# dordanino12/unet-convlstm

Hardware: AMD Instinct MI355X
Metric: training frames/sec, Moving-MNIST 64x64 seq-20 (higher is better)
Workload: dtype bf16; 1 GPU; TemporalUNetDualView(base_ch=64, use_skip_lstm=True) train step, 64x64 seq-20, per-GPU batch 32, AdamW+clip; global_batch=32, seq_len=20, parallelism=dp1

## Files before the change

include/uclstm.h:

```cpp
#ifndef UCLSTM_H
#define UCLSTM_H

#include <stdint.h>

#ifdef __cplusplus
extern "C" {
#endif

#define UCLSTM_ABI_VERSION 16

#define UCLSTM_OK            0
#define UCLSTM_E_BADARG     -1
#define UCLSTM_E_LAUNCH     -2
#define UCLSTM_E_NODEVICE   -3

#define UCLSTM_ACT_TYPE_BF16 0
#define UCLSTM_ACT_TYPE_F16  1


typedef struct {
    const void* ptr;
    int32_t C;
    int32_t Hs, Ws;
    int32_t offY, offX;
// ... 156 lines not shown

int32_t uclstm_bn_bwd_param_grads(const float* sums, int32_t groups, int32_t Cp, int32_t C, float* dgamma, float* dbeta,
                                  int32_t accumulate, void* stream);

int32_t uclstm_maxpool2_fwd(const void* a, void* p, int32_t n_img, int32_t H, int32_t W, int32_t Cp, void* stream);
int32_t uclstm_maxpool2_bwd(const void* a, const void* dp, const void* add, void* da, int32_t n_img, int32_t H, int32_t W, int32_t Cp,
                            void* stream);

int32_t uclstm_splitk_finish(const float* pre, int32_t nslab, int64_t slab, int32_t ld, const float* bias, const float* col_scale,
                             const float* col_shift, int32_t relu, void* out, int64_t pixels, int32_t C, void* stream);

int32_t uclstm_lstm_bwd_pointwise(const void* gates, const float* c_prev, const float* c_new,
                                  const void* dh_a, const void* dh_b, int32_t dh_b_is_f32 ,
                                  int32_t dh_b_nslab , int64_t dh_b_slab ,
                                  float* dc_io, int32_t dc_is_zero, void* dgates, int64_t pixels, int32_t Hd_p, void* stream);
int32_t uclstm_lstm_fwd_pointwise(float* pre, int32_t nslab ,
                                  int64_t slab ,
                                  int32_t clear ,
                                  const float* pre_add ,
                                  const float* bias, const float* c_prev, float* c_out, void* h_out,
                                  void* gates_out, int64_t pixels, int32_t Hd_p, void* stream);
typedef struct {
    float* pre;
    const float* pre_add;
    const float* bias;
    const float* c_prev;
    float* c_out;
    void* h_out;
    void* gates_out;
    int64_t slab;
// ... 154 lines not shown
```

unet-convlstm_amd/_lib.py:

```python
from __future__ import annotations

import ctypes as C
import os
import re

import torch

HERE = os.path.dirname(os.path.abspath(__file__))
LIB_PATH = os.environ.get("UCLSTM_LIB") or os.path.join(HERE, "libuclstm.so")
HEADER_PATH = os.path.join(HERE, "..", "include", "uclstm.h")

ABI_VERSION = 16
EPI_STORE, EPI_LSTM, EPI_ATOMIC = 0, 1, 2
NMODE_IDENTITY, NMODE_LSTM, NMODE_TAPMAJOR = 0, 1, 2
KMODE_IDENTITY, KMODE_GATES, KMODE_IM2COL = 0, 1, 2
ACT_TYPE_BF16, ACT_TYPE_F16 = 0, 1

_ERRORS = {-1: "bad argument (shape/alignment/null contract)", -2: "kernel launch failed", -3: "no gfx950 device"}


class UclstmError(RuntimeError):
    pass


# ... 24 lines not shown

class WgradDesc(C.Structure):
    _fields_ = [("n_img", C.c_int32), ("H", C.c_int32), ("W", C.c_int32),
                ("ktap", C.c_int32), ("scale", C.c_int32), ("pad", C.c_int32), ("nsrc", C.c_int32),
                ("src", Src * 2),
                ("N", C.c_int32), ("Ktot", C.c_int32),
                ("nseg", C.c_int32), ("seg", Seg * 4),
                ("dwp", C.c_void_p), ("splits", C.c_int32), ("accumulate", C.c_int32), ("overlapped", C.c_int32), ("reserved_", C.c_int32),
                ("slab", C.c_int64)]


class LstmFwdPwArgs(C.Structure):
    _fields_ = [("pre", C.c_void_p), ("pre_add", C.c_void_p), ("bias", C.c_void_p), ("c_prev", C.c_void_p), ("c_out", C.c_void_p),
                ("h_out", C.c_void_p), ("gates_out", C.c_void_p), ("slab", C.c_int64), ("pixels", C.c_int64),
                ("nslab", C.c_int32), ("clear", C.c_int32), ("Hd_p", C.c_int32), ("reserved_", C.c_int32)]


class PackDesc(C.Structure):
    _fields_ = [("N", C.c_int32), ("Ktot", C.c_int32), ("taps", C.c_int32), ("nsrc", C.c_int32),
                ("kseg", C.c_int32 * 2), ("cvalid", C.c_int32 * 2), ("choff", C.c_int32 * 2),
                ("n_mode", C.c_int32), ("n_valid", C.c_int32), ("n_cp", C.c_int32),
                ("k_mode", C.c_int32), ("k_hdp", C.c_int32), ("k_hd", C.c_int32),
                ("tap_flip", C.c_int32),
                ("stride_n", C.c_int64), ("stride_k", C.c_int64), ("stride_tap", C.c_int64),
                ("stride_ntap", C.c_int64)]


class PackJob(C.Structure):
    _fields_ = [("d", PackDesc), ("w", C.c_void_p), ("wp", C.c_void_p),
                ("block0", C.c_int32), ("nblocks", C.c_int32), ("gx", C.c_int32), ("family", C.c_int32),
# ... 48 lines not shown
    "uclstm_bn_bwd_apply": [_P, _P, _P, _P, _P, _P, _P, _P, _L, _L, _I, _P],
    "uclstm_bn_pool_bwd_rows": [_L, _I, _I, _I, _I],
    "uclstm_bn_apply_relu_pool": [_P, _P, _P, _P, _P, _L, _I, _I, _I, _I, _P],
    "uclstm_bn_pool_bwd_reduce": [_P, _P, _P, _P, _P, _P, _P, _P, _P, _L, _I, _I, _I, _I, _P],
    "uclstm_bn_pool_bwd_apply": [_P, _P, _P, _P, _P, _P, _P, _P, _P, _L, _I, _I, _I, _I, _P],
    "uclstm_bn_head_fwd": [_P, _P, _P, _P, _P, _P, _L, _L, _I, _I, _P],
    "uclstm_bn_head_bwd_reduce": [_P, _P, _P, _P, _P, _P, _P, _P, _P, _P, _P, _L, _L, _I, _I, _P],
    "uclstm_bn_head_bwd_reduce_ordered": [_P, _P, _P, _P, _P, _P, _P, _P, _P, _P, _P, _P, _L, _L, _I, _I, _I, _P],
    "uclstm_bn_head_bwd_apply": [_P, _P, _P, _P, _P, _P, _P, _P, _P, _L, _L, _I, _I, _P],
    "uclstm_bn_bwd_param_grads": [_P, _I, _I, _I, _P, _P, _I, _P],
    "uclstm_maxpool2_fwd": [_P, _P, _I, _I, _I, _I, _P],
    "uclstm_maxpool2_bwd": [_P, _P, _P, _P, _I, _I, _I, _I, _P],
    "uclstm_lstm_bwd_pointwise": [_P, _P, _P, _P, _P, _I, _I, _L, _P, _I, _P, _L, _I, _P],
    "uclstm_lstm_fwd_pointwise": [_P, _I, _L, _I, _P, _P, _P, _P, _P, _P, _L, _I, _P],
    "uclstm_lstm_fwd_pointwise_group": [C.POINTER(LstmFwdPwArgs), _I, _P],
    "uclstm_splitk_finish": [_P, _I, _L, _I, _P, _P, _P, _I, _P, _L, _I, _P],
    "uclstm_nchw_to_nhwc": [_P, _P, _I, _I, _I, _I, _I, _I, _L, _L, _P],
    "uclstm_nhwc_to_nchw": [_P, _P, _I, _I, _I, _I, _I, _P],
    "uclstm_nchw_grad_to_nhwc": [_P, _P, _I, _I, _I, _I, _I, _P],
    "uclstm_im2col3x3_first": [_P, _P, _I, _I, _I, _I, _I, _I, _L, _L, _P],
    "uclstm_nchw_to_nhwc_f32": [_P, _P, _I, _I, _I, _I, _I, _P],
    "uclstm_nhwc_to_nchw_f32": [_P, _P, _I, _I, _I, _I, _I, _P],
    "uclstm_outconv_fwd": [_P, _P, _P, _P, _L, _I, _I, _I, _I, _P],
    "uclstm_outconv_bwd": [_P, _P, _P, _P, _P, _P, _L, _I, _I, _I, _I, _P],
    "uclstm_outconv_bwd_ordered_rows": [_L, _I],
    "uclstm_outconv_bwd_ordered": [_P, _P, _P, _P, _P, _P, _P, _I, _L, _I, _I, _I, _I, _I, _P],
    "uclstm_colsum": [_P, _P, _L, _I, _P],
    "uclstm_colsum_ordered_rows": [_L, _I],
    "uclstm_colsum_ordered": [_P, _P, _P, _L, _I, _I, _I, _P],
    "uclstm_ordered_sum_f32": [_P, _I, _I, _P, _I, _P],
# ... 107 lines not shown
```

unet-convlstm_amd/csrc/igemm_fwd.hip:

```cpp
#include "common.h"
#include <cstdlib>
#include <type_traits>

namespace {

constexpr int BK = 64;

constexpr uint32_t OOB = 0x80000000u;

struct Derived {
    int Mg;
    int tpg;
    int n_mtiles;
    int n_ntiles;
    int kseg0, kseg1;
    int ksteps;
    int ksplit;
    int kper;
    FastDiv dHW, dW;
    FastDiv dPHW, dW2;
    uint32_t xbias[2];
    uint32_t xbytes[2];
    uint32_t wbytes;
    int strip;
// ... 598 lines not shown
    int n;
    int first[GROUP_MAX + 1];
    int nblk[GROUP_MAX];
    uclstm_igemm_desc d[GROUP_MAX];
    Derived dv[GROUP_MAX];
};

template <int NSRC>
__global__ __launch_bounds__(Shape<2>::NT, 1) void igemm_fwd_group_kernel(const FwdGroup g) {
    const int b = (int)blockIdx.x;
#define UCLSTM_GROUP_MEMBER(j_)                                                                            \
    if (j_ < g.n && b >= g.first[j_] && b < g.first[j_ + 1]) {                                             \
        const int bid = b - g.first[j_];                                                                   \
        if (bid >= g.nblk[j_]) return;                                                                     \
        if (g.d[j_].epi == UCLSTM_EPI_LSTM) igemm_fwd_body<UCLSTM_EPI_LSTM, 2, NSRC>(g.d[j_], g.dv[j_], bid);   \
        else igemm_fwd_body<UCLSTM_EPI_ATOMIC, 2, NSRC>(g.d[j_], g.dv[j_], bid);                           \
        return;                                                                                            \
    }
    UCLSTM_GROUP_MEMBER(0)
    UCLSTM_GROUP_MEMBER(1)
    UCLSTM_GROUP_MEMBER(2)
    UCLSTM_GROUP_MEMBER(3)
#undef UCLSTM_GROUP_MEMBER
}


constexpr int C64_WBYTES = 9 * 64 * 128;
constexpr int C64_ROW = 66 * 128;
constexpr int C64_SLOTS = 10;
constexpr int C64_RED = C64_WBYTES + C64_SLOTS * C64_ROW;
constexpr int C64_SMEM = C64_RED + 4 * 64 * 2 * 4;
// ... 460 lines not shown

static int32_t fwd_group_run(const uclstm_igemm_desc* descs, int32_t n, void* stream, int query) {
    if (!descs || n < 1 || n > GROUP_MAX) return UCLSTM_E_BADARG;
    FwdGroup g{};
    int64_t work[GROUP_MAX];
    int order[GROUP_MAX];
    Derived dvs[GROUP_MAX];
    int64_t nblks[GROUP_MAX];
    for (int i = 0; i < n; ++i) {
        const uclstm_igemm_desc& d = descs[i];
        int shp = 0;
        int64_t mg = 0;
        const int32_t rc = plan_fwd(d, dvs[i], shp, nblks[i], mg);
        if (rc != UCLSTM_OK) return rc;
        if (shp != 2 || (c64_ok(d) && mg % 256 == 0)) return UCLSTM_E_BADARG;
        if (d.epi != UCLSTM_EPI_LSTM && d.epi != UCLSTM_EPI_ATOMIC) return UCLSTM_E_BADARG;
        if (d.nsrc != descs[0].nsrc) return UCLSTM_E_BADARG;
        work[i] = dvs[i].kper;
        order[i] = i;
    }
    for (int a = 1; a < n; ++a)
        for (int b = a; b > 0 && work[order[b]] > work[order[b - 1]]; --b) { const int t = order[b]; order[b] = order[b - 1]; order[b - 1] = t; }
    g.n = n;
    int64_t at = 0;
    for (int k = 0; k < n; ++k) {
        const int i = order[k];
        g.first[k] = (int)at;
        g.nblk[k] = (int)nblks[i];
        g.d[k] = descs[i];
        g.dv[k] = dvs[i];
        at += (nblks[i] + 7) / 8 * 8;
// ... 21 lines not shown
```

unet-convlstm_amd/csrc/pointwise.hip:

```cpp
#include "common.h"
#include <algorithm>
#include <cstdlib>

namespace {

constexpr int NT = 256;

__device__ __forceinline__ void unpack8(const uint4 u, float (&f)[8]) {
    Pack16 p;
    p.u = u;
#pragma unroll
    for (int i = 0; i < 8; ++i) f[i] = act_to_f32(p.e[i]);
}
__device__ __forceinline__ uint4 pack8(const float (&f)[8]) {
    Pack16 p;
#pragma unroll
    for (int i = 0; i < 8; ++i) p.e[i] = f32_to_act(f[i]);
    return p.u;
}
__device__ __forceinline__ float act16_product(float a, float b) {
    float p = a * b;
#ifdef UCLSTM_ACT_F16
    asm("" : "+v"(p));
#endif
// ... 1008 lines not shown
    FastDiv dq[PW_GROUP_MAX];
};
__global__ void lstm_fwd_pw_group_kernel(const LstmFwdPwGroup g) {
    const int b = (int)blockIdx.x;
#pragma unroll
    for (int j = 0; j < PW_GROUP_MAX; ++j) {
        if (j < g.n && b >= g.first[j] && b < g.first[j + 1]) {
            const uclstm_lstm_fwd_pw_args& a = g.a[j];
            lstm_fwd_pw_body(a.pre, a.nslab, a.slab, a.clear, a.pre_add, a.bias, a.c_prev, a.c_out, (act16*)a.h_out, (act16*)a.gates_out,
                             a.pixels * (a.Hd_p / 4), g.dq[j], a.Hd_p, 64 * ((a.Hd_p + 15) / 16), b - g.first[j], g.first[j + 1] - g.first[j]);
            return;
        }
    }
}

__global__ void nchw_to_nhwc_kernel(const float* __restrict__ x, uint4* __restrict__ out, int64_t items, int C, int cpc, FastDiv dHW,
                                    FastDiv dcpc, FastDiv dinner, int64_t inner_stride, int64_t outer_stride) {
    const int HW = dHW.d;
    for (int64_t idx = (int64_t)blockIdx.x * NT + threadIdx.x; idx < items; idx += (int64_t)gridDim.x * NT) {
        const uint32_t t = fdiv((uint32_t)idx, dHW);
        const uint32_t pix = (uint32_t)idx - t * HW;
        const uint32_t img = fdiv(t, dcpc);
        const uint32_t cc = t - img * cpc;
        const uint32_t o = fdiv(img, dinner);
        const uint32_t in = img - o * dinner.d;
        const float* src = x + (int64_t)in * outer_stride + (int64_t)o * inner_stride;
        float v[8];
#pragma unroll
        for (int i = 0; i < 8; ++i) {
            const int c = cc * 8 + i;
// ... 847 lines not shown
                  (act16*)gates_out, items, make_fastdiv(Hd_p / 4), Hd_p, N);
    return UCLSTM_OK;
}

extern "C" int32_t uclstm_lstm_bwd_pointwise(const void* gates, const float* c_prev, const float* c_new, const void* dh_a,
                                             const void* dh_b, int32_t dh_b_is_f32, int32_t dh_b_nslab, int64_t dh_b_slab, float* dc_io,
                                             int32_t dc_is_zero, void* dgates, int64_t pixels, int32_t Hd_p, void* stream) {
    if (!lstm_bwd_pw_ok(gates, c_prev, c_new, dh_a, dh_b, dh_b_is_f32, dh_b_nslab, dh_b_slab, dc_io, dgates, pixels, Hd_p)) return UCLSTM_E_BADARG;
    const int64_t chunks = pixels * (Hd_p / 8);
    UCLSTM_LAUNCH(lstm_bwd_pw_kernel, dim3(ew_grid(chunks)), dim3(NT), 0, (hipStream_t)stream, (const uint4*)gates, c_prev, c_new,
                       (const uint4*)dh_a, dh_b, dh_b_is_f32, dh_b_nslab, dh_b_slab, dc_io, dc_is_zero, (uint4*)dgates, chunks,
                       make_fastdiv(Hd_p / 8));
    return UCLSTM_OK;
}

extern "C" int32_t uclstm_nchw_to_nhwc(const float* x, void* out, int32_t n_img, int32_t C, int32_t Cp, int32_t H, int32_t W,
                                       int32_t inner, int64_t inner_stride, int64_t outer_stride, void* stream) {
    if (!x || !aligned16(out) || n_img <= 0 || C <= 0 || Cp < C || (Cp % 8) || H <= 0 || W <= 0 || inner <= 0 || (n_img % inner))
        return UCLSTM_E_BADARG;
    const int64_t items = (int64_t)n_img * (Cp / 8) * H * W;
    if (items >= ((int64_t)1 << 31)) return UCLSTM_E_BADARG;
    UCLSTM_LAUNCH(nchw_to_nhwc_kernel, dim3(ew_grid(items)), dim3(NT), 0, (hipStream_t)stream, x, (uint4*)out, items, C, Cp / 8,
                       make_fastdiv(H * W), make_fastdiv(Cp / 8), make_fastdiv(inner), inner_stride, outer_stride);
    return UCLSTM_OK;
}

extern "C" int32_t uclstm_nchw_grad_to_nhwc(const float* g, void* out, int32_t n_img, int32_t C, int32_t Cp, int32_t H, int32_t W,
                                            void* stream) {
    return uclstm_nchw_to_nhwc(g, out, n_img, C, Cp, H, W, n_img, 0, (int64_t)C * H * W, stream);
}
// ... 278 lines not shown
```

unet-convlstm_amd/modules.py:

```python
from __future__ import annotations

from typing import List, Optional, Sequence, Tuple

import torch
import torch.nn as nn

from . import ops
from ._lib import UclstmError

Tensor = torch.Tensor


def _need_grad(*ts) -> bool:
    return torch.is_grad_enabled() and any(t is not None and t.requires_grad for t in ts)


class ConvLSTMCell(nn.Module):

    def __init__(self, input_dim, hidden_dim, kernel_size=3, bias=True):
        super().__init__()
        if kernel_size % 2 == 0 or not 1 <= kernel_size <= 7:
            raise UclstmError("ConvLSTMCell: kernel_size must be odd and <= 7")
        padding = kernel_size // 2
        self.input_dim = input_dim
# ... 292 lines not shown
            st = []
            for s in state:
                if s is None or s[0] is None:
                    st.append(None)
                else:
                    st.append((ops.ToNHWC.apply(s[0].contiguous().float()), ops.StateToNHWC.apply(s[1].contiguous().float())))
        grouped = False
        if self.use_skip_lstm and len(self.temporal.layers) == 1:
            cells = (self.temporal.layers[0], self.lstm_skip3.layers[0], self.lstm_skip2.layers[0])
            h0, c0 = (None, None) if (st is None or st[0] is None) else st[0]
            members = [(seq(xb), h0, c0), (seq(x3), None, None), (seq(x2), None, None)]
            full = [(xs, hh, cc, cl.conv.weight, cl.conv.bias, cl.hidden_dim, cl.input_dim) for (xs, hh, cc), cl in zip(members, cells)]
            if ops.convlstm_group_ok(full):
                needs = [_need_grad(*f[:5]) for f in full]
                pre = ops.convlstm_group_forward(full, any(needs))
                outs = [ops.ConvLSTMSeqPre.apply(*f, nd, hh, ch, gt) for f, nd, (hh, ch, gt) in zip(full, needs, pre)]
                b_all, new_st = outs[0][0], [(outs[0][0][-1], outs[0][1])]
                x3_l, x2_l = outs[1][0], outs[2][0]
                grouped = True
        if not grouped:
            b_all, new_st = self.temporal.seq_nhwc(seq(xb), st)
            if self.use_skip_lstm:
                x3_l, _ = self.lstm_skip3.seq_nhwc(seq(x3), None)
                x2_l, _ = self.lstm_skip2.seq_nhwc(seq(x2), None)
        if self.use_skip_lstm:
            x3 = x3_l.reshape(T * B, *x3_l.shape[2:])
            x2 = x2_l.reshape(T * B, *x2_l.shape[2:])
        b_flat = b_all.reshape(T * B, *b_all.shape[2:])

        d3 = self.up3.forward_nhwc(b_flat, x3, c * 8, T)
        d2 = self.up2.forward_nhwc(d3, x2, c * 4, T)
# ... 48 lines not shown
```

unet-convlstm_amd/ops.py:

```python
from __future__ import annotations

import ctypes as C
import os
from typing import List, Optional, Sequence, Tuple

import torch

from . import _lib as L

BF16 = torch.bfloat16
F16 = torch.float16
F32 = torch.float32
ACT = (BF16, F16)

_COMPUTE_DTYPE = BF16


def set_compute_dtype(dtype) -> None:
    global _COMPUTE_DTYPE
    if dtype not in ACT:
        raise L.UclstmError(f"compute dtype must be torch.bfloat16 or torch.float16, got {dtype}")
    _COMPUTE_DTYPE = dtype


# ... 128 lines not shown
    return C.c_void_p(torch.cuda.current_stream().cuda_stream)


def _dev(t: torch.Tensor, dtype=None, what: str = "tensor") -> torch.Tensor:
    if not isinstance(t, torch.Tensor) or not t.is_cuda:
        raise L.UclstmError(f"{what}: a HIP device tensor is required (this package has no CPU path)")
    if dtype is not None and (t.dtype not in dtype if isinstance(dtype, tuple) else t.dtype != dtype):
        raise L.UclstmError(f"{what}: expected {dtype}, got {t.dtype}")
    if not t.is_contiguous():
        raise L.UclstmError(f"{what}: must be contiguous")
    return t


def _p(t: Optional[torch.Tensor]):
    return None if t is None else C.c_void_p(t.data_ptr())


PROFILE: Optional[list] = None


SHAPE_LOG: Optional[list] = None
KERNEL_LOG: Optional[list] = None


LAUNCH_LOG: Optional[list] = None


def _log_shape(d) -> None:
    if SHAPE_LOG is not None or KERNEL_LOG is not None or LAUNCH_LOG is not None:
        shp = int(L.lib.uclstm_igemm_fwd_shape(C.byref(d)))
# ... 498 lines not shown


def _schedule_join(device) -> None:
    key = str(device)
    if key in _JOIN_PENDING:
        return
    _JOIN_PENDING.add(key)

    def join():
        _JOIN_PENDING.discard(key)
        torch.cuda.current_stream(device).wait_stream(side_stream(device))

    torch.autograd.Variable._execution_engine.queue_callback(join)


def wgrad_into_param(weight: torch.Tensor, desc: L.PackDesc, inputs: Sequence[torch.Tensor], run_gemm) -> Optional[torch.Tensor]:
    g = weight.grad
    if not (ASYNC_WGRAD and g is not None and g.dtype == F32 and g.is_contiguous() and g.shape == weight.shape):
        return unpack_wgrad(desc, run_gemm(), weight)
    dev = weight.device
    main, side = torch.cuda.current_stream(dev), side_stream(dev)
    side.wait_stream(main)
    global _WGRAD_OVERLAPPED
    with torch.cuda.stream(side):
        _WGRAD_OVERLAPPED = True
        try:
            dwp = run_gemm()
        finally:
            _WGRAD_OVERLAPPED = False
        _unpack_wgrad_launch(desc, dwp, g, 1)
        for t in inputs:
            if t is not None:
                t.record_stream(side)
# ... 201 lines not shown

def igemm_group(items, K, kind: str = "igemm_fwd_group") -> None:
    arr = (L.IgemmDesc * len(items))(*[it[0] for it in items])
    for it in items:
        _log_shape(it[0])
    _timed(kind + "[patch128x256]" if PROFILE is not None else kind, sum(it[1] for it in items),
           lambda: L.check(K.uclstm_igemm_fwd_group(arr, len(items), _stream()), "igemm_fwd_group"),
           " | ".join(it[3] for it in items), nbytes=sum(it[2] for it in items))


def group_launchable(descs) -> bool:
    arr = (L.IgemmDesc * len(descs))(*descs)
    return int(L.lib.uclstm_igemm_fwd_group_blocks(arr, len(descs))) > 0


def igemm_wgrad(srcs: Sequence[SrcView], dy_segs, N: int, Ktot: int, out_hw: Tuple[int, int], n_img: int, *, ktap: int, scale: int = 1,
                pad: int = 0) -> torch.Tensor:
    dev = srcs[0].t.device
    _same_act_dtype([sv.t for sv in srcs] + [sg[0] for sg in dy_segs], "igemm_wgrad")
    K = _k(srcs[0].t)
    per_img = max([_bytes_per_img(sv.t) for sv in srcs] + [_bytes_per_img(sg[0]) for sg in dy_segs])
    chunks = _img_chunks(n_img, 1, per_img, "igemm_wgrad")
    descs = []
    for i0, i1 in chunks:
        d = L.WgradDesc()
        d.n_img, d.H, d.W = i1 - i0, out_hw[0], out_hw[1]
        d.ktap, d.scale, d.pad, d.nsrc = ktap, scale, pad, len(srcs)
        for i, sv in enumerate(srcs):
            (sv if len(chunks) == 1 else SrcView(sv.t[i0:i1], sv.offY, sv.offX)).fill(d.src[i])
        d.N, d.Ktot = N, Ktot
        d.nseg = len(dy_segs)
        for i, sg in enumerate(dy_segs):
            _fill_seg(d.seg[i], *(sg if len(chunks) == 1 else (sg[0][i0:i1],) + tuple(sg[1:])))
        d.splits, d.accumulate, d.slab = 0, 1, N * Ktot
        d.overlapped = int(_WGRAD_OVERLAPPED)
        splits = int(L.lib.uclstm_igemm_wgrad_splits(C.byref(d)))
        if splits < 1:
            raise L.UclstmError(f"igemm_wgrad: bad descriptor (code {splits})")
        d.splits = splits
        descs.append(d)
    if LAUNCH_LOG is not None:
        if len(chunks) > 1:
            LAUNCH_LOG.append(("split", "igemm_wgrad", len(chunks)))
        for d in descs:
            LAUNCH_LOG.append(("wgrad", int(L.lib.uclstm_igemm_wgrad_shape(C.byref(d))), N, Ktot, int(d.splits)))
    total = sum(d.splits for d in descs)
    dwp = torch.empty((total, N, Ktot), dtype=F32, device=dev)
    taps = ktap * ktap
    at = 0
    for d in descs:
        d.dwp = dwp[at].data_ptr()
        at += d.splits
        flops = 2.0 * d.n_img * out_hw[0] * out_hw[1] * N * taps * sum(s.t.shape[3] for s in srcs)
        kind = "igemm_wgrad"
        if PROFILE is not None:
            kind += "[" + {4: "ring64", 3: "p3_256x256", 2: "p2_128x128", 1: "p2_64x256", 0: "generic"}.get(int(L.lib.uclstm_igemm_wgrad_shape(C.byref(d))), "?") + "]"
        _timed(kind, flops, lambda d=d: L.check(K.uclstm_igemm_wgrad(C.byref(d), _stream()), "igemm_wgrad"),
               f"M={d.n_img * out_hw[0] * out_hw[1]} N={N} K={Ktot} ktap={ktap} splits={d.splits}",
               nbytes=(_nb(*[sv.t for sv in srcs], *[sg[0] for sg in dy_segs]) * (d.n_img / n_img) + 4.0 * N * Ktot) if PROFILE is not None else 0.0)
    return dwp


def colsum(a: torch.Tensor, into: Optional[torch.Tensor] = None) -> torch.Tensor:
    _dev(a, ACT, "colsum input")
    Cp = a.shape[-1]
    if _DETERMINISTIC:
        pixels = a.numel() // Cp
        out = into if into is not None else torch.empty((Cp,), dtype=F32, device=a.device)
        partials = torch.empty((int(L.lib.uclstm_colsum_ordered_rows(pixels, Cp)), Cp), dtype=F32, device=a.device)
        _log_reduce("colsum_ordered")
        L.check(L.lib.uclstm_colsum_ordered(_p(a), _p(partials), _p(out), pixels, Cp, 1 if into is not None else 0, L.act_type(a.dtype),
                                            _stream()), "colsum_ordered")
        return out
    out = into if into is not None else torch.zeros((Cp,), dtype=F32, device=a.device)
# ... 585 lines not shown
        N, H, W, Cp = x.shape
        k = weight.shape[-1]
        dx = torch.empty_like(x)
        scratch = torch.empty((3 * N * H * W + 2,), dtype=F32, device=x.device)
        need_w = ctx.needs_input_grad[1]
        g = direct_grad(weight) if need_w else None
        dw = g if g is not None else (torch.empty_like(weight) if need_w else None)
        L.check(_k(x).uclstm_attention_bwd(_p(x), _p(dout), _p(weight), _p(att), _p(desc), _p(arg), _p(dx), _p(dw), int(g is not None),
                                           _p(scratch), N, H, W, Cp, ctx.channels, k, _stream()), "attention_bwd")
        if g is not None:
            grad_written(weight)
            return dx, None, None
        return dx, dw, None


class ConvLSTMSeq(torch.autograd.Function):

    @staticmethod
    def forward(ctx, x_all, h0, c0, weight, bias, Hd, Cx, need_grad, out=None):
        ctx.set_materialize_grads(False)
        _dev(x_all, ACT, "x_all")
        adt = x_all.dtype
        K = _k(x_all)
        T, B, H, W, Cxp = x_all.shape
        Hdp = cpad(Hd)
        dev = x_all.device
        ks = weight.shape[-1]
        pd = lstm_pack_desc(Hd, Cx, ks)
        bp = pack_bias(pd, bias) if bias is not None else None
        if out is not None:
# ... 84 lines not shown
        need_h0 = ctx.needs_input_grad[1]
        for t in range(T - 1, -1, -1):
            c_prev = c_hist[t] if (has_c0 or t > 0) else None
            L.check(K.uclstm_lstm_bwd_pointwise(_p(gates[t]), _p(c_prev), _p(c_hist[t + 1]),
                                                    _p(dh_all[t]) if dh_all is not None else None, _p(dh_rec),
                                                    1 if ksplit > 1 else 0, nsl, pixels * Hdp, _p(dc),
                                                    int(dc_zero), _p(dgates[t]), pixels, Hdp, _stream()), "lstm_bwd_pointwise")
            dc_zero = False
            if t > 0 or need_h0:
                dh_rec = buf[t & 1]
                if ksplit > 1:
                    igemm_atomic([SrcView(dgates[t])], wd_h, (H, W), B, dh_rec.view(nsl, pixels, Hdp), ksplit, ktap=ks, pad=ks // 2,
                                 slabs=True)
                else:
                    igemm_store([SrcView(dgates[t])], wd_h, (H, W), B, [(dh_rec, 0, ddh.N, 0, 1, 0, 0)], ktap=ks, pad=ks // 2)
        dg_flat = dgates.view(T * B, H, W, 4 * Hdp)
        x_flat = x_all.reshape(T * B, H, W, Cxp)
        hprev_flat = h_hist[:T].reshape(T * B, H, W, Hdp)
        dweight = None
        if ctx.needs_input_grad[3]:
            ud = lstm_wgrad_unpack_desc(Hd, Cx, ks)
            dweight = wgrad_into_param(weight, ud, [x_all, h_hist, dgates],
                                       lambda: igemm_wgrad([SrcView(x_flat), SrcView(hprev_flat)], [(dg_flat, 0, 4 * Hdp, 0, 1, 0, 0)],
                                                           ud.N, ud.Ktot, (H, W), T * B, ktap=ks, pad=ks // 2))
        dbias = None
        if has_bias and ctx.needs_input_grad[4]:
            if Hdp == Hd:
                dbias = bias_grad_from_colsum(dg_flat, bias, 4 * Hd)
            else:
                dbias = colsum(dg_flat).view(4, Hdp)[:, :Hd].reshape(4 * Hd).contiguous()
        dx_all = None
        if ctx.needs_input_grad[0]:
            ddx = lstm_dgrad_pack_desc(Hd, Cx, Cx, ks)
            wd_x = pack_weights(ddx, weight, 0, adt)
            dx_all = torch.empty_like(x_all)
            igemm_store([SrcView(dg_flat)], wd_x, (H, W), T * B, [(dx_all.view(T * B, H, W, Cxp), 0, ddx.N, 0, 1, 0, 0)], ktap=ks,
                        pad=ks // 2)
        dh0 = (dh_rec if dh_rec.dtype == adt else dh_rec.sum(dim=0).to(adt)) if need_h0 else None
        dc0 = dc if (has_c0 and ctx.needs_input_grad[2]) else None
        return dx_all, dh0, dc0, dweight, dbias, None, None, None


GROUP_LSTM = os.environ.get("UCLSTM_GROUP_LSTM", "1") != "0"
FUSE_POOL = os.environ.get("UCLSTM_FUSE_POOL", "1") != "0"
FUSE_HEAD = os.environ.get("UCLSTM_FUSE_HEAD", "1") != "0"
_GROUP_PLANS: dict = {}
_CUS = 256
_BLOCK_OVERHEAD_STEPS = 12.0


def _lpt_makespan(blocks: List[Tuple[float, int]], cus: int = _CUS) -> float:
    import heapq
    free = [0.0] * cus
    for dur, cnt in sorted(blocks, reverse=True):
# ... 138 lines not shown
    @staticmethod
    def forward(ctx, x_all, h0, c0, weight, bias, Hd, Cx, need_grad, h_hist, c_hist, gates):
        ctx.set_materialize_grads(False)
        T = x_all.shape[0]
        if need_grad:
            ctx.save_for_backward(x_all, weight, h_hist, c_hist, gates, bias)
            ctx.cfg = (Hd, Cx, c0 is not None, bias is not None, weight.shape[-1])
            note_use(weight, bias)
        return h_hist[1:], c_hist[T]

    @staticmethod
    def backward(ctx, dh_all, dc_T):
        return ConvLSTMSeq.backward(ctx, dh_all, dc_T) + (None, None, None)


def convlstm_group_ok(members) -> bool:
    if not GROUP_LSTM or len(members) < 2 or len(members) > 4:
        return False
    x0 = members[0][0]
    try:
        descs = []
        for x_all, h0, c0, weight, bias, Hd, Cx in members:
            if x_all.dim() != 5 or x_all.shape[0] != x0.shape[0] or x_all.shape[1] != x0.shape[1] or x_all.dtype != x0.dtype:
                return False
            if weight.shape[-1] != 3 or cpad(Hd) != Hd or Hd % 64 or x_all.shape[4] % 64 or (x_all.shape[1] * x_all.shape[2] * x_all.shape[3]) % 256:
                return False
            T, B, H, W, Cxp = x_all.shape
            pd = lstm_pack_desc(Hd, Cx, 3)
            d = L.IgemmDesc()
            d.n_img, d.H, d.W, d.groups = B, H, W, 1
# ... 52 lines not shown
```

Baseline: 20510 frames/s.

## Group ConvLSTM backward across layers with batched pointwise, dh igemm, and chunked overlapped wgrad

Adds a grouped backward autograd function for the ConvLSTM layers that were already grouped in forward. At each timestep it runs one combined pointwise-backward kernel for all members and one grouped igemm (with store or atomic split-K epilogues) for the recurrent dh. It also launches weight-gradient GEMMs in time chunks on a side stream as the dgates for each chunk become ready. The aim is fewer per-timestep launches and overlap of wgrad with the serial recurrence, at the cost of more complex scheduling, stream synchronization and extra scratch memory.

```diff
diff --git a/include/uclstm.h b/include/uclstm.h
--- a/include/uclstm.h
+++ b/include/uclstm.h
@@ -194,6 +194,19 @@
                                   const void* dh_a, const void* dh_b, int32_t dh_b_is_f32 ,
                                   int32_t dh_b_nslab , int64_t dh_b_slab ,
                                   float* dc_io, int32_t dc_is_zero, void* dgates, int64_t pixels, int32_t Hd_p, void* stream);
+typedef struct {
+    const void* gates;
+    const float* c_prev;
+    const float* c_new;
+    const void* dh_a;
+    const void* dh_b;
+    float* dc_io;
+    void* dgates;
+    int64_t dh_b_slab;
+    int64_t pixels;
+    int32_t dh_b_is_f32, dh_b_nslab, dc_is_zero, Hd_p;
+} uclstm_lstm_bwd_pw_args;
+int32_t uclstm_lstm_bwd_pointwise_group(const uclstm_lstm_bwd_pw_args* args, int32_t n, int32_t act_type, void* stream);
 int32_t uclstm_lstm_fwd_pointwise(float* pre, int32_t nslab ,
                                   int64_t slab ,
                                   int32_t clear ,
diff --git a/unet-convlstm_amd/_lib.py b/unet-convlstm_amd/_lib.py
--- a/unet-convlstm_amd/_lib.py
+++ b/unet-convlstm_amd/_lib.py
@@ -62,6 +62,12 @@
     _fields_ = [("pre", C.c_void_p), ("pre_add", C.c_void_p), ("bias", C.c_void_p), ("c_prev", C.c_void_p), ("c_out", C.c_void_p),
                 ("h_out", C.c_void_p), ("gates_out", C.c_void_p), ("slab", C.c_int64), ("pixels", C.c_int64),
                 ("nslab", C.c_int32), ("clear", C.c_int32), ("Hd_p", C.c_int32), ("reserved_", C.c_int32)]
+
+
+class LstmBwdPwArgs(C.Structure):
+    _fields_ = [("gates", C.c_void_p), ("c_prev", C.c_void_p), ("c_new", C.c_void_p), ("dh_a", C.c_void_p), ("dh_b", C.c_void_p),
+                ("dc_io", C.c_void_p), ("dgates", C.c_void_p), ("dh_b_slab", C.c_int64), ("pixels", C.c_int64),
+                ("dh_b_is_f32", C.c_int32), ("dh_b_nslab", C.c_int32), ("dc_is_zero", C.c_int32), ("Hd_p", C.c_int32)]
 
 
 class PackDesc(C.Structure):
@@ -140,6 +146,7 @@
     "uclstm_lstm_bwd_pointwise": [_P, _P, _P, _P, _P, _I, _I, _L, _P, _I, _P, _L, _I, _P],
     "uclstm_lstm_fwd_pointwise": [_P, _I, _L, _I, _P, _P, _P, _P, _P, _P, _L, _I, _P],
     "uclstm_lstm_fwd_pointwise_group": [C.POINTER(LstmFwdPwArgs), _I, _P],
+    "uclstm_lstm_bwd_pointwise_group": [C.POINTER(LstmBwdPwArgs), _I, _I, _P],
     "uclstm_splitk_finish": [_P, _I, _L, _I, _P, _P, _P, _I, _P, _L, _I, _P],
     "uclstm_nchw_to_nhwc": [_P, _P, _I, _I, _I, _I, _I, _I, _L, _L, _P],
     "uclstm_nhwc_to_nchw": [_P, _P, _I, _I, _I, _I, _I, _P],
diff --git a/unet-convlstm_amd/csrc/igemm_fwd.hip b/unet-convlstm_amd/csrc/igemm_fwd.hip
--- a/unet-convlstm_amd/csrc/igemm_fwd.hip
+++ b/unet-convlstm_amd/csrc/igemm_fwd.hip
@@ -636,7 +636,9 @@
         const int bid = b - g.first[j_];                                                                   \
         if (bid >= g.nblk[j_]) return;                                                                     \
         if (g.d[j_].epi == UCLSTM_EPI_LSTM) igemm_fwd_body<UCLSTM_EPI_LSTM, 2, NSRC>(g.d[j_], g.dv[j_], bid);   \
-        else igemm_fwd_body<UCLSTM_EPI_ATOMIC, 2, NSRC>(g.d[j_], g.dv[j_], bid);                           \
+        else if (NSRC == 1 && g.d[j_].epi == UCLSTM_EPI_STORE) {                                           \
+            if constexpr (NSRC == 1) igemm_fwd_body<UCLSTM_EPI_STORE, 2, 1>(g.d[j_], g.dv[j_], bid);       \
+        } else igemm_fwd_body<UCLSTM_EPI_ATOMIC, 2, NSRC>(g.d[j_], g.dv[j_], bid);                         \
         return;                                                                                            \
     }
     UCLSTM_GROUP_MEMBER(0)
@@ -1127,7 +1129,8 @@
         const int32_t rc = plan_fwd(d, dvs[i], shp, nblks[i], mg);
         if (rc != UCLSTM_OK) return rc;
         if (shp != 2 || (c64_ok(d) && mg % 256 == 0)) return UCLSTM_E_BADARG;
-        if (d.epi != UCLSTM_EPI_LSTM && d.epi != UCLSTM_EPI_ATOMIC) return UCLSTM_E_BADARG;
+        const bool store_ok = d.epi == UCLSTM_EPI_STORE && d.nsrc == 1 && !d.stats;
+        if (d.epi != UCLSTM_EPI_LSTM && d.epi != UCLSTM_EPI_ATOMIC && !store_ok) return UCLSTM_E_BADARG;
         if (d.nsrc != descs[0].nsrc) return UCLSTM_E_BADARG;
         work[i] = dvs[i].kper;
         order[i] = i;
diff --git a/unet-convlstm_amd/csrc/pointwise.hip b/unet-convlstm_amd/csrc/pointwise.hip
--- a/unet-convlstm_amd/csrc/pointwise.hip
+++ b/unet-convlstm_amd/csrc/pointwise.hip
@@ -1046,6 +1046,26 @@
     }
 }
 
+struct LstmBwdPwGroup {
+    int n;
+    int first[PW_GROUP_MAX + 1];
+    uclstm_lstm_bwd_pw_args a[PW_GROUP_MAX];
+    FastDiv dcpc[PW_GROUP_MAX];
+};
+__global__ void lstm_bwd_pw_group_kernel(const LstmBwdPwGroup g) {
+    const int b = (int)blockIdx.x;
+#pragma unroll
+    for (int j = 0; j < PW_GROUP_MAX; ++j) {
+        if (j < g.n && b >= g.first[j] && b < g.first[j + 1]) {
+            const uclstm_lstm_bwd_pw_args& a = g.a[j];
+            lstm_bwd_pw_body((const uint4*)a.gates, a.c_prev, a.c_new, (const uint4*)a.dh_a, a.dh_b, a.dh_b_is_f32, a.dh_b_nslab, a.dh_b_slab,
+                             a.dc_io, a.dc_is_zero, (uint4*)a.dgates, a.pixels * (a.Hd_p / 8), g.dcpc[j], b - g.first[j],
+                             g.first[j + 1] - g.first[j]);
+            return;
+        }
+    }
+}
+
 __global__ void nchw_to_nhwc_kernel(const float* __restrict__ x, uint4* __restrict__ out, int64_t items, int C, int cpc, FastDiv dHW,
                                     FastDiv dcpc, FastDiv dinner, int64_t inner_stride, int64_t outer_stride) {
     const int HW = dHW.d;
@@ -1923,6 +1943,45 @@
     return UCLSTM_OK;
 }
 
+__attribute__((visibility("hidden"))) int32_t UCLSTM_ACT_IMPL(lstm_bwd_pointwise_group)(const uclstm_lstm_bwd_pw_args* args, int32_t n,
+                                                                                       void* stream) {
+    if (!args || n < 1 || n > PW_GROUP_MAX) return UCLSTM_E_BADARG;
+    int order[PW_GROUP_MAX];
+    for (int i = 0; i < n; ++i) {
+        const uclstm_lstm_bwd_pw_args& a = args[i];
+        if (!lstm_bwd_pw_ok(a.gates, a.c_prev, a.c_new, a.dh_a, a.dh_b, a.dh_b_is_f32, a.dh_b_nslab, a.dh_b_slab, a.dc_io, a.dgates, a.pixels,
+                            a.Hd_p))
+            return UCLSTM_E_BADARG;
+        order[i] = i;
+    }
+    for (int x = 1; x < n; ++x)
+        for (int y = x; y > 0 && args[order[y]].pixels * (args[order[y]].Hd_p / 8) > args[order[y - 1]].pixels * (args[order[y - 1]].Hd_p / 8); --y) {
+            const int t = order[y]; order[y] = order[y - 1]; order[y - 1] = t;
+        }
+    LstmBwdPwGroup g{};
+    g.n = n;
+    int64_t at = 0;
+    for (int k = 0; k < n; ++k) {
+        const uclstm_lstm_bwd_pw_args& a = args[order[k]];
+        g.a[k] = a;
+        g.dcpc[k] = make_fastdiv(a.Hd_p / 8);
+        g.first[k] = (int)at;
+        at += ew_grid(a.pixels * (a.Hd_p / 8));
+    }
+    if (at > 0x7fffffff) return UCLSTM_E_BADARG;
+    for (int k = n; k <= PW_GROUP_MAX; ++k) g.first[k] = (int)at;
+    UCLSTM_LAUNCH(lstm_bwd_pw_group_kernel, dim3((unsigned)at), dim3(NT), 0, (hipStream_t)stream, g);
+    return UCLSTM_OK;
+}
+#ifndef UCLSTM_ACT_F16
+int32_t lstm_bwd_pointwise_group_impl_f16(const uclstm_lstm_bwd_pw_args*, int32_t, void*);
+extern "C" int32_t uclstm_lstm_bwd_pointwise_group(const uclstm_lstm_bwd_pw_args* args, int32_t n, int32_t act_type, void* stream) {
+    if (act_type == UCLSTM_ACT_TYPE_BF16) return UCLSTM_ACT_IMPL(lstm_bwd_pointwise_group)(args, n, stream);
+    if (act_type == UCLSTM_ACT_TYPE_F16) return lstm_bwd_pointwise_group_impl_f16(args, n, stream);
+    return UCLSTM_E_BADARG;
+}
+#endif
+
 extern "C" int32_t uclstm_nchw_to_nhwc(const float* x, void* out, int32_t n_img, int32_t C, int32_t Cp, int32_t H, int32_t W,
                                        int32_t inner, int64_t inner_stride, int64_t outer_stride, void* stream) {
     if (!x || !aligned16(out) || n_img <= 0 || C <= 0 || Cp < C || (Cp % 8) || H <= 0 || W <= 0 || inner <= 0 || (n_img % inner))
diff --git a/unet-convlstm_amd/modules.py b/unet-convlstm_amd/modules.py
--- a/unet-convlstm_amd/modules.py
+++ b/unet-convlstm_amd/modules.py
@@ -330,7 +330,10 @@
             if ops.convlstm_group_ok(full):
                 needs = [_need_grad(*f[:5]) for f in full]
                 pre = ops.convlstm_group_forward(full, any(needs))
-                outs = [ops.ConvLSTMSeqPre.apply(*f, nd, hh, ch, gt) for f, nd, (hh, ch, gt) in zip(full, needs, pre)]
+                if all(needs):
+                    outs = ops.convlstm_group_apply(full, pre)
+                else:
+                    outs = [ops.ConvLSTMSeqPre.apply(*f, nd, hh, ch, gt) for f, nd, (hh, ch, gt) in zip(full, needs, pre)]
                 b_all, new_st = outs[0][0], [(outs[0][0][-1], outs[0][1])]
                 x3_l, x2_l = outs[1][0], outs[2][0]
                 grouped = True
diff --git a/unet-convlstm_amd/ops.py b/unet-convlstm_amd/ops.py
--- a/unet-convlstm_amd/ops.py
+++ b/unet-convlstm_amd/ops.py
@@ -166,6 +166,16 @@
 
 def _p(t: Optional[torch.Tensor]):
     return None if t is None else C.c_void_p(t.data_ptr())
+
+
+POISON_SCRATCH = os.environ.get("UCLSTM_POISON_SCRATCH", "0") == "1"
+
+
+def _scratch(shape, dtype, device) -> torch.Tensor:
+    t = torch.empty(shape, dtype=dtype, device=device)
+    if POISON_SCRATCH:
+        t.fill_(float("nan"))
+    return t
 
 
 PROFILE: Optional[list] = None
@@ -694,9 +704,14 @@
     torch.autograd.Variable._execution_engine.queue_callback(join)
 
 
+def wgrad_goes_to_side(weight: torch.Tensor) -> bool:
+    g = weight.grad
+    return bool(ASYNC_WGRAD and g is not None and g.dtype == F32 and g.is_contiguous() and g.shape == weight.shape)
+
+
 def wgrad_into_param(weight: torch.Tensor, desc: L.PackDesc, inputs: Sequence[torch.Tensor], run_gemm) -> Optional[torch.Tensor]:
     g = weight.grad
-    if not (ASYNC_WGRAD and g is not None and g.dtype == F32 and g.is_contiguous() and g.shape == weight.shape):
+    if not wgrad_goes_to_side(weight):
         return unpack_wgrad(desc, run_gemm(), weight)
     dev = weight.device
     main, side = torch.cuda.current_stream(dev), side_stream(dev)
@@ -928,50 +943,78 @@
     return int(L.lib.uclstm_igemm_fwd_group_blocks(arr, len(descs))) > 0
 
 
-def igemm_wgrad(srcs: Sequence[SrcView], dy_segs, N: int, Ktot: int, out_hw: Tuple[int, int], n_img: int, *, ktap: int, scale: int = 1,
-                pad: int = 0) -> torch.Tensor:
-    dev = srcs[0].t.device
+class _WgradPlan:
+    pass
+
+
+def wgrad_plan(srcs: Sequence[SrcView], dy_segs, N: int, Ktot: int, out_hw: Tuple[int, int], ranges: Sequence[Tuple[int, int]], *, ktap: int,
+               scale: int = 1, pad: int = 0, overlapped: Optional[bool] = None) -> _WgradPlan:
     _same_act_dtype([sv.t for sv in srcs] + [sg[0] for sg in dy_segs], "igemm_wgrad")
-    K = _k(srcs[0].t)
     per_img = max([_bytes_per_img(sv.t) for sv in srcs] + [_bytes_per_img(sg[0]) for sg in dy_segs])
-    chunks = _img_chunks(n_img, 1, per_img, "igemm_wgrad")
-    descs = []
-    for i0, i1 in chunks:
-        d = L.WgradDesc()
-        d.n_img, d.H, d.W = i1 - i0, out_hw[0], out_hw[1]
-        d.ktap, d.scale, d.pad, d.nsrc = ktap, scale, pad, len(srcs)
-        for i, sv in enumerate(srcs):
-            (sv if len(chunks) == 1 else SrcView(sv.t[i0:i1], sv.offY, sv.offX)).fill(d.src[i])
-        d.N, d.Ktot = N, Ktot
-        d.nseg = len(dy_segs)
-        for i, sg in enumerate(dy_segs):
-            _fill_seg(d.seg[i], *(sg if len(chunks) == 1 else (sg[0][i0:i1],) + tuple(sg[1:])))
-        d.splits, d.accumulate, d.slab = 0, 1, N * Ktot
-        d.overlapped = int(_WGRAD_OVERLAPPED)
-        splits = int(L.lib.uclstm_igemm_wgrad_splits(C.byref(d)))
-        if splits < 1:
-            raise L.UclstmError(f"igemm_wgrad: bad descriptor (code {splits})")
-        d.splits = splits
-        descs.append(d)
-    if LAUNCH_LOG is not None:
-        if len(chunks) > 1:
-            LAUNCH_LOG.append(("split", "igemm_wgrad", len(chunks)))
+    n_all = srcs[0].t.shape[0]
+    pl = _WgradPlan()
+    pl.srcs, pl.dy_segs, pl.N, pl.Ktot, pl.out_hw, pl.ktap = list(srcs), list(dy_segs), N, Ktot, out_hw, ktap
+    pl.K, pl.dev, pl.n_img, pl.dwp = _k(srcs[0].t), srcs[0].t.device, sum(i1 - i0 for i0, i1 in ranges), None
+    pl.ranges = []
+    for r0, r1 in ranges:
+        chunks = [(r0 + i0, r0 + i1) for i0, i1 in _img_chunks(r1 - r0, 1, per_img, "igemm_wgrad")]
+        descs = []
+        for i0, i1 in chunks:
+            whole = i0 == 0 and i1 == n_all
+            d = L.WgradDesc()
+            d.n_img, d.H, d.W = i1 - i0, out_hw[0], out_hw[1]
+            d.ktap, d.scale, d.pad, d.nsrc = ktap, scale, pad, len(srcs)
+            for i, sv in enumerate(srcs):
+                (sv if whole else SrcView(sv.t[i0:i1], sv.offY, sv.offX)).fill(d.src[i])
+            d.N, d.Ktot = N, Ktot
+            d.nseg = len(dy_segs)
+            for i, sg in enumerate(dy_segs):
+                _fill_seg(d.seg[i], *(sg if whole else (sg[0][i0:i1],) + tuple(sg[1:])))
+            d.splits, d.accumulate, d.slab = 0, 1, N * Ktot
+            d.overlapped = int(_WGRAD_OVERLAPPED if overlapped is None else overlapped)
+            splits = int(L.lib.uclstm_igemm_wgrad_splits(C.byref(d)))
+            if splits < 1:
+                raise L.UclstmError(f"igemm_wgrad: bad descriptor (code {splits})")
+            d.splits = splits
+            descs.append(d)
+        if LAUNCH_LOG is not None:
+            if len(chunks) > 1:
+                LAUNCH_LOG.append(("split", "igemm_wgrad", len(chunks)))
+            for d in descs:
+                LAUNCH_LOG.append(("wgrad", int(L.lib.uclstm_igemm_wgrad_shape(C.byref(d))), N, Ktot, int(d.splits)))
+        pl.ranges.append(descs)
+    pl.total = sum(d.splits for descs in pl.ranges for d in descs)
+    return pl
+
+
+def wgrad_alloc(pl: _WgradPlan) -> torch.Tensor:
+    pl.dwp = _scratch((pl.total, pl.N, pl.Ktot), F32, pl.dev)
+    at = 0
+    for descs in pl.ranges:
         for d in descs:
-            LAUNCH_LOG.append(("wgrad", int(L.lib.uclstm_igemm_wgrad_shape(C.byref(d))), N, Ktot, int(d.splits)))
-    total = sum(d.splits for d in descs)
-    dwp = torch.empty((total, N, Ktot), dtype=F32, device=dev)
-    taps = ktap * ktap
-    at = 0
-    for d in descs:
-        d.dwp = dwp[at].data_ptr()
-        at += d.splits
+            d.dwp = pl.dwp[at].data_ptr()
+            at += d.splits
+    return pl.dwp
+
+
+def wgrad_launch_range(pl: _WgradPlan, i: int) -> None:
+    taps = pl.ktap * pl.ktap
+    srcs, dy_segs, N, Ktot, out_hw = pl.srcs, pl.dy_segs, pl.N, pl.Ktot, pl.out_hw
+    for d in pl.ranges[i]:
         flops = 2.0 * d.n_img * out_hw[0] * out_hw[1] * N * taps * sum(s.t.shape[3] for s in srcs)
         kind = "igemm_wgrad"
         if PROFILE is not None:
             kind += "[" + {4: "ring64", 3: "p3_256x256", 2: "p2_128x128", 1: "p2_64x256", 0: "generic"}.get(int(L.lib.uclstm_igemm_wgrad_shape(C.byref(d))), "?") + "]"
-        _timed(kind, flops, lambda d=d: L.check(K.uclstm_igemm_wgrad(C.byref(d), _stream()), "igemm_wgrad"),
-               f"M={d.n_img * out_hw[0] * out_hw[1]} N={N} K={Ktot} ktap={ktap} splits={d.splits}",
-               nbytes=(_nb(*[sv.t for sv in srcs], *[sg[0] for sg in dy_segs]) * (d.n_img / n_img) + 4.0 * N * Ktot) if PROFILE is not None else 0.0)
+        _timed(kind, flops, lambda d=d: L.check(pl.K.uclstm_igemm_wgrad(C.byref(d), _stream()), "igemm_wgrad"),
+               f"M={d.n_img * out_hw[0] * out_hw[1]} N={N} K={Ktot} ktap={pl.ktap} splits={d.splits}",
+               nbytes=(_nb(*[sv.t for sv in srcs], *[sg[0] for sg in dy_segs]) * (d.n_img / srcs[0].t.shape[0]) + 4.0 * N * Ktot) if PROFILE is not None else 0.0)
+
+
+def igemm_wgrad(srcs: Sequence[SrcView], dy_segs, N: int, Ktot: int, out_hw: Tuple[int, int], n_img: int, *, ktap: int, scale: int = 1,
+                pad: int = 0) -> torch.Tensor:
+    pl = wgrad_plan(srcs, dy_segs, N, Ktot, out_hw, [(0, n_img)], ktap=ktap, scale=scale, pad=pad)
+    dwp = wgrad_alloc(pl)
+    wgrad_launch_range(pl, 0)
     return dwp
 
 
@@ -1587,6 +1630,38 @@
         return dx, dw, None
 
 
+def _lstm_bwd_finish(x_all, weight, bias, h_hist, dgates, dh_rec, dc, cfg, needs, weight_done: bool = False):
+    Hd, Cx, has_c0, has_bias, ks = cfg
+    T, B, H, W, Cxp = x_all.shape
+    Hdp = cpad(Hd)
+    adt = x_all.dtype
+    dg_flat = dgates.view(T * B, H, W, 4 * Hdp)
+    x_flat = x_all.reshape(T * B, H, W, Cxp)
+    hprev_flat = h_hist[:T].reshape(T * B, H, W, Hdp)
+    dweight = None
+    if needs[3] and not weight_done:
+        ud = lstm_wgrad_unpack_desc(Hd, Cx, ks)
+        dweight = wgrad_into_param(weight, ud, [x_all, h_hist, dgates],
+                                   lambda: igemm_wgrad([SrcView(x_flat), SrcView(hprev_flat)], [(dg_flat, 0, 4 * Hdp, 0, 1, 0, 0)],
+                                                       ud.N, ud.Ktot, (H, W), T * B, ktap=ks, pad=ks // 2))
+    dbias = None
+    if has_bias and needs[4]:
+        if Hdp == Hd:
+            dbias = bias_grad_from_colsum(dg_flat, bias, 4 * Hd)
+        else:
+            dbias = colsum(dg_flat).view(4, Hdp)[:, :Hd].reshape(4 * Hd).contiguous()
+    dx_all = None
+    if needs[0]:
+        ddx = lstm_dgrad_pack_desc(Hd, Cx, Cx, ks)
+        wd_x = pack_weights(ddx, weight, 0, adt)
+        dx_all = torch.empty_like(x_all)
+        igemm_store([SrcView(dg_flat)], wd_x, (H, W), T * B, [(dx_all.view(T * B, H, W, Cxp), 0, ddx.N, 0, 1, 0, 0)], ktap=ks,
+                    pad=ks // 2)
+    dh0 = (dh_rec if dh_rec.dtype == adt else dh_rec.sum(dim=0).to(adt)) if needs[1] else None
+    dc0 = dc if (has_c0 and needs[2]) else None
+    return dx_all, dh0, dc0, dweight, dbias
+
+
 class ConvLSTMSeq(torch.autograd.Function):
 
     @staticmethod
@@ -1701,30 +1776,7 @@
                                  slabs=True)
                 else:
                     igemm_store([SrcView(dgates[t])], wd_h, (H, W), B, [(dh_rec, 0, ddh.N, 0, 1, 0, 0)], ktap=ks, pad=ks // 2)
-        dg_flat = dgates.view(T * B, H, W, 4 * Hdp)
-        x_flat = x_all.reshape(T * B, H, W, Cxp)
-        hprev_flat = h_hist[:T].reshape(T * B, H, W, Hdp)
-        dweight = None
-        if ctx.needs_input_grad[3]:
-            ud = lstm_wgrad_unpack_desc(Hd, Cx, ks)
-            dweight = wgrad_into_param(weight, ud, [x_all, h_hist, dgates],
-                                       lambda: igemm_wgrad([SrcView(x_flat), SrcView(hprev_flat)], [(dg_flat, 0, 4 * Hdp, 0, 1, 0, 0)],
-                                                           ud.N, ud.Ktot, (H, W), T * B, ktap=ks, pad=ks // 2))
-        dbias = None
-        if has_bias and ctx.needs_input_grad[4]:
-            if Hdp == Hd:
-                dbias = bias_grad_from_colsum(dg_flat, bias, 4 * Hd)
-            else:
-                dbias = colsum(dg_flat).view(4, Hdp)[:, :Hd].reshape(4 * Hd).contiguous()
-        dx_all = None
-        if ctx.needs_input_grad[0]:
-            ddx = lstm_dgrad_pack_desc(Hd, Cx, Cx, ks)
-            wd_x = pack_weights(ddx, weight, 0, adt)
-            dx_all = torch.empty_like(x_all)
-            igemm_store([SrcView(dg_flat)], wd_x, (H, W), T * B, [(dx_all.view(T * B, H, W, Cxp), 0, ddx.N, 0, 1, 0, 0)], ktap=ks,
-                        pad=ks // 2)
-        dh0 = (dh_rec if dh_rec.dtype == adt else dh_rec.sum(dim=0).to(adt)) if need_h0 else None
-        dc0 = dc if (has_c0 and ctx.needs_input_grad[2]) else None
+        dx_all, dh0, dc0, dweight, dbias = _lstm_bwd_finish(x_all, weight, bias, h_hist, dgates, dh_rec, dc, ctx.cfg, ctx.needs_input_grad[:5])
         return dx_all, dh0, dc0, dweight, dbias, None, None, None
 
 
@@ -1893,6 +1945,211 @@
         return ConvLSTMSeq.backward(ctx, dh_all, dc_T) + (None, None, None)
 
 
+GROUP_LSTM_BWD = os.environ.get("UCLSTM_GROUP_LSTM_BWD", "0") != "0"
+
+
+def parse_wgrad_chunks(text: str, n: int = 3) -> Tuple[int, ...]:
+    parts = [p.strip() for p in str(text).split(",")]
+    try:
+        vals = [int(p) for p in parts]
+    except ValueError:
+        raise L.UclstmError(f"UCLSTM_LSTM_WGRAD_CHUNKS: expected a number or {n} comma-separated numbers, got {text!r}") from None
+    if len(vals) == 1:
+        vals = vals * n
+    if len(vals) != n or any(v < 1 for v in vals):
+        raise L.UclstmError(f"UCLSTM_LSTM_WGRAD_CHUNKS: expected a number or {n} comma-separated numbers >= 1, got {text!r}")
+    return tuple(vals)
+
+
+LSTM_WGRAD_CHUNKS = parse_wgrad_chunks(os.environ.get("UCLSTM_LSTM_WGRAD_CHUNKS", "1,1,2"))
+
+
+def plan_time_chunks(T: int, chunks: int) -> List[Tuple[int, int]]:
+    n = max(1, min(int(chunks), T))
+    edges = [(i * T) // n for i in range(n + 1)]
+    return [(edges[i], edges[i + 1]) for i in range(n - 1, -1, -1)]
+
+
+def _bwd_member_shape(Hd: int, pixels: int) -> Tuple[int, int]:
+    return ((Hd + 127) // 128) * (pixels // 256), 4 * Hd // 64
+
+
+def _dh_desc(m, t: int, dh_rec: torch.Tensor):
+    if m.ksplit > 1:
+        return _atomic_desc([SrcView(m.dgates[t])], m.wd_h, (m.H, m.W), m.B, dh_rec.view(m.nsl, m.pixels, m.Hdp), m.ksplit, ktap=3, pad=1,
+                            slabs=True)
+    d = L.IgemmDesc()
+    d.n_img, d.H, d.W, d.groups = m.B, m.H, m.W, 1
+    d.ktap, d.scale, d.pad, d.nsrc = 3, 1, 1, 1
+    SrcView(m.dgates[t]).fill(d.src[0])
+    d.wp, d.N, d.Ktot = m.wd_h.data_ptr(), m.wd_h.shape[0], m.wd_h.shape[1]
+    d.relu, d.epi, d.nseg = 0, L.EPI_STORE, 1
+    _fill_seg(d.seg[0], dh_rec, 0, d.N, 0, 1, 0, 0)
+    _same_act_dtype([m.dgates, m.wd_h, dh_rec], "igemm_fwd(store)")
+    flops = 2.0 * m.pixels * d.N * 9 * m.dgates.shape[-1]
+    nbytes = _nb(m.dgates[t], m.wd_h, dh_rec) if PROFILE is not None else 0.0
+    return d, flops, nbytes, f"M={m.pixels} N={d.N} K={d.Ktot} ktap=3 store"
+
+
+def convlstm_group_bwd_ok(members) -> bool:
+    if not GROUP_LSTM_BWD or len(members) < 2 or len(members) > 4:
+        return False
+    try:
+        shapes = [_bwd_member_shape(Hd, x_all.shape[1] * x_all.shape[2] * x_all.shape[3]) for x_all, _, _, _, _, Hd, _ in members]
+        plan = plan_group_ksplit(shapes)
+        descs = []
+        for (x_all, h0, c0, weight, bias, Hd, Cx), ks in zip(members, plan):
+            T, B, H, W, _ = x_all.shape
+            pd = lstm_dgrad_pack_desc(Hd, Cx, Hd, 3)
+            d = L.IgemmDesc()
+            d.n_img, d.H, d.W, d.groups = B, H, W, 1
+            d.ktap, d.scale, d.pad, d.nsrc = 3, 1, 1, 1
+            d.src[0].ptr, d.src[0].C, d.src[0].Hs, d.src[0].Ws = x_all.data_ptr(), 4 * Hd, H, W
+            d.wp, d.N, d.Ktot = x_all.data_ptr(), pd.N, pd.Ktot
+            if ks > 1:
+                d.epi, d.acc_out, d.acc_ld, d.ksplit, d.acc_slab = L.EPI_ATOMIC, x_all.data_ptr(), Hd, ks, B * H * W * Hd
+            else:
+                d.epi, d.nseg = L.EPI_STORE, 1
+                sg = d.seg[0]
+                sg.ptr, sg.n_begin, sg.n_end, sg.C, sg.c_off, sg.Hd, sg.Wd, sg.scale = x_all.data_ptr(), 0, pd.N, Hd, 0, H, W, 1
+            descs.append(d)
+        return group_launchable(descs)
+    except Exception:
+        return False
+
+
+class ConvLSTMGroupSeq(torch.autograd.Function):
+    PER = 8
+
+    @staticmethod
+    def forward(ctx, cfg, *flat):
+        ctx.set_materialize_grads(False)
+        n = len(flat) // ConvLSTMGroupSeq.PER
+        outs, saved, cfgs = [], [], []
+        for i in range(n):
+            x_all, h0, c0, weight, bias, h_hist, c_hist, gates = flat[i * ConvLSTMGroupSeq.PER:(i + 1) * ConvLSTMGroupSeq.PER]
+            Hd, Cx = cfg["dims"][i]
+            saved += [x_all, weight, h_hist, c_hist, gates, bias]
+            cfgs.append((Hd, Cx, c0 is not None, bias is not None, weight.shape[-1]))
+            note_use(weight, bias)
+            outs += [h_hist[1:], c_hist[x_all.shape[0]]]
+        ctx.save_for_backward(*saved)
+        ctx.cfgs, ctx.ksplit, ctx.chunks = cfgs, cfg.get("ksplit"), cfg.get("chunks")
+        return tuple(outs)
+
+    @staticmethod
+    def backward(ctx, *grads):
+        n = len(ctx.cfgs)
+        PER = ConvLSTMGroupSeq.PER
+        ms = []
+        for i in range(n):
+            m = _LstmMember()
+            m.x_all, m.weight, m.h_hist, m.c_hist, m.gates, m.bias = ctx.saved_tensors[i * 6:(i + 1) * 6]
+            m.cfg = ctx.cfgs[i]
+            m.Hd, m.Cx, m.has_c0, m.has_bias, _ = m.cfg
+            m.needs = ctx.needs_input_grad[1 + i * PER:1 + i * PER + 5]
+            m.T, m.B, m.H, m.W, m.Cxp = m.x_all.shape
+            m.Hdp, m.pixels = cpad(m.Hd), m.B * m.H * m.W
+            m.dh_all = None if grads[2 * i] is None else grads[2 * i].contiguous()
+            m.dc_T = grads[2 * i + 1]
+            ms.append(m)
+        T, adt, dev = ms[0].T, ms[0].x_all.dtype, ms[0].x_all.device
+        K = _k(ms[0].x_all)
+        plan = ctx.ksplit if ctx.ksplit is not None else plan_group_ksplit([_bwd_member_shape(m.Hd, m.pixels) for m in ms])
+        nchunks = ctx.chunks if ctx.chunks is not None else (LSTM_WGRAD_CHUNKS + (LSTM_WGRAD_CHUNKS[-1],) * n)[:n]
+        main = torch.cuda.current_stream(dev)
+        for m, ks, nch in zip(ms, plan, nchunks):
+            m.dgates = _scratch((T, m.B, m.H, m.W, 4 * m.Hdp), adt, dev)
+            m.dc = torch.empty((m.B, m.H, m.W, m.Hdp), dtype=F32, device=dev)
+            m.dc_zero = m.dc_T is None
+            if not m.dc_zero:
+                m.dc.copy_(m.dc_T)
+            ddh = lstm_dgrad_pack_desc(m.Hd, m.Cx, m.Hd, 3)
+            m.wd_h = pack_weights(ddh, m.weight, m.Cx * 9, adt)
+            m.ksplit = int(ks)
+            m.nsl = ksplit_used(ddh.Ktot, m.ksplit, 3) if m.ksplit > 1 else 1
+            shape = (m.nsl, m.B, m.H, m.W, m.Hdp) if m.ksplit > 1 else (m.B, m.H, m.W, m.Hdp)
+            m.buf = [_scratch(shape, F32 if m.ksplit > 1 else adt, dev) for _ in range(2)]
+            m.dh_rec = None
+            m.chunked = bool(m.needs[3]) and wgrad_goes_to_side(m.weight)
+            if m.chunked:
+                m.tchunks = plan_time_chunks(T, nch)
+                m.ud = lstm_wgrad_unpack_desc(m.Hd, m.Cx, 3)
+                m.wplan = wgrad_plan([SrcView(m.x_all.reshape(T * m.B, m.H, m.W, m.Cxp)), SrcView(m.h_hist[:T].reshape(T * m.B, m.H, m.W, m.Hdp))],
+                                     [(m.dgates.view(T * m.B, m.H, m.W, 4 * m.Hdp), 0, 4 * m.Hdp, 0, 1, 0, 0)], m.ud.N, m.ud.Ktot, (m.H, m.W),
+                                     [(t0 * m.B, t1 * m.B) for t0, t1 in m.tchunks], ktap=3, pad=1, overlapped=True)
+                if LAUNCH_LOG is not None:
+                    LAUNCH_LOG.append(("lstm_wgrad_chunks", ms.index(m), tuple(m.tchunks)))
+        side = side_stream(dev) if any(m.chunked for m in ms) else None
+        global _WGRAD_OVERLAPPED
+        for t in range(T - 1, -1, -1):
+            pws = []
+            for m in ms:
+                c_prev = m.c_hist[t] if (m.has_c0 or t > 0) else None
+                a = L.LstmBwdPwArgs()
+                a.gates, a.c_prev, a.c_new = m.gates[t].data_ptr(), None if c_prev is None else c_prev.data_ptr(), m.c_hist[t + 1].data_ptr()
+                a.dh_a = None if m.dh_all is None else m.dh_all[t].data_ptr()
+                a.dh_b = None if m.dh_rec is None else m.dh_rec.data_ptr()
+                a.dh_b_is_f32, a.dh_b_nslab, a.dh_b_slab = (1 if m.ksplit > 1 else 0), m.nsl, m.pixels * m.Hdp
+                a.dc_io, a.dc_is_zero, a.dgates = m.dc.data_ptr(), int(m.dc_zero), m.dgates[t].data_ptr()
+                a.pixels, a.Hd_p = m.pixels, m.Hdp
+                m.dc_zero = False
+                pws.append(a)
+            if LAUNCH_LOG is not None:
+                LAUNCH_LOG.append(("group", "lstm_bwd_pointwise", n))
+            arr = (L.LstmBwdPwArgs * n)(*pws)
+            L.check(L.lib.uclstm_lstm_bwd_pointwise_group(arr, n, L.act_type(adt), _stream()), "lstm_bwd_pointwise_group")
+            for m in ms:
+                if m.chunked:
+                    for ci, (t0, t1) in enumerate(m.tchunks):
+                        if t0 != t:
+                            continue
+                        side.wait_stream(main)
+                        with torch.cuda.stream(side):
+                            _WGRAD_OVERLAPPED = True
+                            try:
+                                if m.wplan.dwp is None:
+                                    wgrad_alloc(m.wplan)
+                                wgrad_launch_range(m.wplan, ci)
+                            finally:
+                                _WGRAD_OVERLAPPED = False
+            items = []
+            for m in ms:
+                if t > 0 or m.needs[1]:
+                    m.dh_rec = m.buf[t & 1]
+                    items.append(_dh_desc(m, t, m.dh_rec))
+            if items:
+                if LAUNCH_LOG is not None:
+                    LAUNCH_LOG.append(("group", "lstm_bwd_dh", len(items)))
+                igemm_group(items, K, kind="igemm_fwd_group_dh")
+        out = [None]
+        for m in ms:
+            if m.chunked:
+                with torch.cuda.stream(side):
+                    _unpack_wgrad_launch(m.ud, m.wplan.dwp, m.weight.grad, 1)
+                    for tns in (m.x_all, m.h_hist, m.dgates):
+                        tns.record_stream(side)
+                    for hook in GRAD_SIDE_HOOKS:
+                        hook(m.weight)
+                _schedule_join(dev)
+            dx_all, dh0, dc0, dweight, dbias = _lstm_bwd_finish(m.x_all, m.weight, m.bias, m.h_hist, m.dgates, m.dh_rec, m.dc, m.cfg, m.needs,
+                                                                weight_done=m.chunked)
+            out += [dx_all, dh0, dc0, dweight, dbias, None, None, None]
+        return tuple(out)
+
+
+def convlstm_group_apply(members, pre, *, ksplit=None, chunks=None):
+    if not convlstm_group_bwd_ok(members):
+        return [ConvLSTMSeqPre.apply(*f, True, hh, ch, gt) for f, (hh, ch, gt) in zip(members, pre)]
+    flat = []
+    for (x_all, h0, c0, weight, bias, Hd, Cx), (hh, ch, gt) in zip(members, pre):
+        flat += [x_all, h0, c0, weight, bias, hh, ch, gt]
+    cfg = {"dims": [(f[5], f[6]) for f in members], "ksplit": None if ksplit is None else tuple(ksplit),
+           "chunks": None if chunks is None else tuple(chunks)}
+    outs = ConvLSTMGroupSeq.apply(cfg, *flat)
+    return [(outs[2 * i], outs[2 * i + 1]) for i in range(len(members))]
+
+
 def convlstm_group_ok(members) -> bool:
     if not GROUP_LSTM or len(members) < 2 or len(members) > 4:
         return False
```

After: 20450 frames/s. No clear change (-0.3%).
